# antoyang/FrozenBiLM

Measured on AMD Instinct MI355X. Metric: video-text samples/sec (MLM fwd+bwd) DeBERTa-XL+adapters, higher is better.
Workload: dtype bf16; 1 GPU; DeBERTa-v2-XLarge(24L)+adapters ds8/8, B=32/GPU, T=10x1024, L=256 (S=266), MLM fwd+bwd+allreduce+clip+Adam, dropout 0.1 live, seeded random weights; global_batch=32, seq_len=266, parallelism=dp1, dead_layer23_encoder_pass=skipped (output unused, SURVEY fact 6); FLOPs still counted

## Files before the change

frozenbilm_amd/csrc/attn_bwd.hip:

```cpp
#include "attn_common.h"
#include "../../include/fbl.h"

namespace {
using namespace attn;

__global__ void rowdot_kernel(const bf16* dO, const bf16* O, long ld, float* out, int B, int S, int nh) {
  const long gid = (long)blockIdx.x * blockDim.x + threadIdx.x;
  const long idx = gid >> 3;
  const int c = (int)(gid & 7);
  const long total = (long)B * S * nh;
  const bool live = idx < total;
  const long row = live ? idx / nh : 0;
  const int h = live ? (int)(idx % nh) : 0;
  float s = 0.f;
  if (live) {
    const bf16x8 x = *(const bf16x8*)(dO + row * ld + h * 64 + c * 8);
    const bf16x8 y = *(const bf16x8*)(O + row * ld + h * 64 + c * 8);
#pragma unroll
    for (int e = 0; e < 8; ++e) s += bf2f(x[e]) * bf2f(y[e]);
  }
  s += __shfl_xor(s, 1, 64);
  s += __shfl_xor(s, 2, 64);
  s += __shfl_xor(s, 4, 64);
  if (live && c == 0) {
// ... 643 lines not shown
      *(bf16x4*)(ok + dt * 16) = (bf16x4){f2bf(dk[dt][0]), f2bf(dk[dt][1]), f2bf(dk[dt][2]), f2bf(dk[dt][3])};
    }
  }
}

struct BwdQArgs {
  const bf16* dS;
  const bf16* k; long ldk;
  const bf16* pkx;
  const int32_t* klen; const int32_t* border;
  bf16* dQ; long lddq;
  int B, S, Sp, nh;
  const int32_t* row0;
};
constexpr int LDG1 = 104;
constexpr int Q_DS = 0;
constexpr int Q_KS = Q_DS + 8192;
constexpr int Q_G1 = Q_KS + 8192;
constexpr int Q_TAB = Q_G1 + 64 * LDG1 * 2;
constexpr int Q_TOTAL = Q_TAB + 16384;
static_assert(3 * Q_TOTAL <= 160 * 1024, "three workgroups per CU");

template <bool PACKED = false>
__global__ __launch_bounds__(256, 3) void attn_bwd_dq_kernel(BwdQArgs a) {
  extern __shared__ __attribute__((aligned(16))) char smem[];
  const int tid = threadIdx.x, lane = tid & 63;
  const int w = __builtin_amdgcn_readfirstlane(tid >> 6);
  const int c = lane & 15, g = lane >> 4;
  const int S = a.S, Sp = a.Sp;
  const WgCoord wc = wg_coord(Sp / 64, a.nh, a.B, a.border);
  const int i0 = wc.x * 64, h = wc.h, b = wc.b;
  const int i = i0 + w * 16 + c;
  const long rb = PACKED ? (long)a.row0[b] : (long)b * S;
  const int lim = PACKED ? min(a.row0[b + 1] - a.row0[b], S) : S;
  const int kl = a.klen ? min(a.klen[b], S) : S;
  const int nkt = (i0 < kl) ? (kl + 63) / 64 : 0;
  const int srow = tid >> 3, sch = tid & 7;
  const int sb = srow * 128 + ((sch ^ tswz(srow)) << 4);
  const int ks0 = (w < 2) ? 0 : 1;
  bf16* g1 = (bf16*)(smem + Q_G1) + (w * 16 + c) * LDG1;
  const int wr = w * 16 + c;
  f32x4 dq[4];
#pragma unroll
  for (int dt = 0; dt < 4; ++dt) dq[dt] = (f32x4){0.f, 0.f, 0.f, 0.f};
  if (nkt > 0) {
    for (int t = tid; t < (64 * LDG1 * 2) / 16; t += 256) *(bf16x8*)(smem + Q_G1 + t * 16) = (bf16x8){0, 0, 0, 0, 0, 0, 0, 0};
    __syncthreads();
  }

  const long sbase = ((long)b * a.nh + h) * Sp * Sp;
  const __amdgpu_buffer_rsrc_t sr = buf_rsrc(a.dS + sbase + (long)i0 * Sp);
  const __amdgpu_buffer_rsrc_t kr = buf_rsrc(a.k + rb * a.ldk + h * 64);
  const __amdgpu_buffer_rsrc_t xr = buf_rsrc(a.pkx + (long)h * 2 * Sp * 64);
  const uint32_t so = (uint32_t)((wr * Sp + g * 16) * 2);
  const uint32_t ldk2 = (uint32_t)(a.ldk * 2);
  const int beta0 = (i0 - 64 + Sp) >> 6;

  struct Regs { bf16x8 s[2], k[2], x[2]; } R;
  auto load_pair = [&](int jt) {
#pragma unroll
    for (int t = 0; t < 2; ++t) {
      R.s[t] = buf_ld16(sr, so + (uint32_t)(t * 16), (uint32_t)(jt * 128));
      const uint32_t jr = (uint32_t)min(jt * 64 + srow + t * 32, lim - 1);
      R.k[t] = buf_ld16(kr, jr * ldk2 + (uint32_t)(sch * 16), 0);
      R.x[t] = buf_ld16(xr, (uint32_t)((srow + t * 32) * 128 + sch * 16), (uint32_t)((beta0 - jt) * 8192));
    }
  };
  if (nkt > 0) {
    load_pair(0);
#pragma unroll
    for (int t = 0; t < 2; ++t)
      *(bf16x8*)(smem + Q_TAB + ((beta0 + 1) & 1) * 8192 + sb + t * 4096) =
          buf_ld16(xr, (uint32_t)((srow + t * 32) * 128 + sch * 16), (uint32_t)((beta0 + 1) * 8192));
  }
  for (int jt = 0; jt < nkt; ++jt) {
#pragma unroll
    for (int t = 0; t < 2; ++t) {
      *(bf16x8*)(smem + Q_KS + sb + t * 4096) = R.k[t];
      *(bf16x8*)(smem + Q_TAB + ((beta0 - jt) & 1) * 8192 + sb + t * 4096) = R.x[t];
      *(bf16x8*)(smem + Q_DS + wr * 128 + (((2 * g + t) ^ (wr & 7)) << 4)) = R.s[t];
    }
    {
      bf16* gs = g1 + wr + 64 - g * 16 - ks0 * 32;
#pragma unroll
      for (int t = 0; t < 2; ++t)
#pragma unroll
        for (int e = 0; e < 8; ++e) gs[-(t * 8 + e)] = R.s[t][e];
    }
    __syncthreads();
    load_pair(min(jt + 1, nkt - 1));
#pragma unroll
    for (int kk = 0; kk < 2; ++kk) {
      const int rk = kk * 32 + g * 8 + (c >> 2);
      const bf16x8 sf = *(const bf16x8*)(smem + Q_DS + wr * 128 + (((kk * 4 + g) ^ (wr & 7)) << 4));
#pragma unroll
      for (int dt = 0; dt < 4; ++dt) {
        const int ch = dt * 2 + ((c >> 1) & 1), sub = (c & 1) * 8;
        union { tr16x4 h[2]; bf16x8 v; } u;
        u.h[0] = lds_tr16((const bf16*)(smem + Q_KS + rk * 128 + ((ch ^ tswz(rk)) << 4) + sub));
        u.h[1] = lds_tr16((const bf16*)(smem + Q_KS + (rk + 4) * 128 + ((ch ^ tswz(rk + 4)) << 4) + sub));
        dq[dt] = __builtin_amdgcn_mfma_f32_16x16x32_bf16(u.v, sf, dq[dt], 0, 0, 0);
      }
    }
#pragma unroll
    for (int u3 = 0; u3 < 3; ++u3) {
      const int x0 = (ks0 + u3) * 32 + g * 8;
      const int slot = ((beta0 - jt + (x0 >> 6)) & 1) * 8192;
      const int r = (x0 & 63) + (c >> 2);
      const bf16x8 gf = *(const bf16x8*)(g1 + u3 * 32 + g * 8);
#pragma unroll
      for (int dt = 0; dt < 4; ++dt) {
        const int ch = dt * 2 + ((c >> 1) & 1), sub = (c & 1) * 8;
        union { tr16x4 h[2]; bf16x8 v; } ut;
        ut.h[0] = lds_tr16((const bf16*)(smem + Q_TAB + slot + r * 128 + ((ch ^ tswz(r)) << 4) + sub));
        ut.h[1] = lds_tr16((const bf16*)(smem + Q_TAB + slot + (r + 4) * 128 + ((ch ^ tswz(r + 4)) << 4) + sub));
        dq[dt] = __builtin_amdgcn_mfma_f32_16x16x32_bf16(ut.v, gf, dq[dt], 0, 0, 0);
      }
    }
    __syncthreads();
  }
  if (i < lim) {
    bf16* op = a.dQ + (rb + i) * a.lddq + h * 64 + g * 4;
#pragma unroll
    for (int dt = 0; dt < 4; ++dt)
      *(bf16x4*)(op + dt * 16) = (bf16x4){f2bf(dq[dt][0]), f2bf(dq[dt][1]), f2bf(dq[dt][2]), f2bf(dq[dt][3])};
  }
}

struct ShearArgs {
  const bf16* X;
  const bf16* YT; long y_sh, y_sb, y_sd;
  const bf16* PT;
  const int16_t* relidx;
  const int32_t* klen;
  const int32_t* border;
  bf16* out; long ldout;
  int B, S, Sp, nh, span2, Wg;
  int lin;
  const int32_t* row0;
};
__device__ __forceinline__ void gt_window(const int16_t* relidx, int S, int kl, int r0, int Wg, int* rbase, int* nks) {
  const int hi = 2 * S - 2;
  const int dlo = -(r0 + 31), dhi = kl - 1 - r0;
  const int rb = (int)relidx[min(max(dlo + S - 1, 0), hi)] & ~7;
  const int rt = (int)relidx[min(max(dhi + S - 1, 0), hi)];
  *rbase = rb;
  *nks = min((rt - rb + 32) / 32, Wg / 32);
}
constexpr int C_IDX = 0;
constexpr int C_G = C_IDX + 2048;

template <bool PACKED = false>
__global__ __launch_bounds__(128) void attn_bwd_shear_kernel(ShearArgs a) {
  extern __shared__ __attribute__((aligned(16))) char smem[];
  const int tid = threadIdx.x, lane = tid & 63;
  const int w = __builtin_amdgcn_readfirstlane(tid >> 6);
  const int c = lane & 15, g = lane >> 4;
  const int S = a.S, Sp = a.Sp;
  const WgCoord wc = wg_coord(Sp / 32, a.nh, a.B, a.border);
  const int r0 = wc.x * 32, h = wc.h, b = wc.b;
  const int LDG = a.Wg + 8;
  const int rl = w * 16 + c;
  const int row = r0 + rl;
  bf16* G = (bf16*)(smem + C_G);
  int16_t* idx = (int16_t*)(smem + C_IDX);
  const bf16x8 z8 = {0, 0, 0, 0, 0, 0, 0, 0};
  const int kl = a.klen ? min(a.klen[b], S) : S;
  const long rb = PACKED ? (long)a.row0[b] : (long)b * S;
  const int lim = PACKED ? min(a.row0[b + 1] - a.row0[b], S) : S;
  if (r0 >= kl) {
    if (row < lim) {
      bf16* op = a.out + (rb + row) * a.ldout + h * 64 + g * 4;
#pragma unroll
      for (int dt = 0; dt < 4; ++dt) *(bf16x4*)(op + dt * 16) = (bf16x4){0, 0, 0, 0};
    }
    return;
  }
  int rbase, nks;
  gt_window(a.relidx, S, kl, r0, a.Wg, &rbase, &nks);
  const int izero = (int)a.relidx[S - 1];
  {
    const int vpr = nks * 4;
    for (int t = tid; t < 32 * vpr; t += 128) *(bf16x8*)(G + (t / vpr) * LDG + (t % vpr) * 8) = z8;
  }
  attn::load_idx_padded(idx, a.relidx, S, Sp, tid, 128);
  const long xbase = (((long)b * a.nh + h) * Sp + row) * Sp;
  f32x4 acc[4];
#pragma unroll
  for (int dt = 0; dt < 4; ++dt) acc[dt] = (f32x4){0.f, 0.f, 0.f, 0.f};
  __syncthreads();

  const int nct = (kl + 63) / 64;
  const bf16* ytb = a.YT + h * a.y_sh + b * a.y_sb + (long)c * a.y_sd + g * 8;
  const int16_t* ib = idx + (Sp - 1 - row + g * 8);
  bf16* grow = G + rl * LDG - rbase;
  const int wmax = rbase + nks * 32 - 1;
  const int dummy = rbase + a.Wg;
  const int lin0 = izero + g * 8 - row;
  const int rw = r0 + w * 16;
  struct Frags { bf16x8 y[8], x[2]; };
  auto load_ct = [&](int ct, Frags& F) {
    const int c0 = ct * 64;
#pragma unroll
    for (int kk = 0; kk < 2; ++kk)
#pragma unroll
      for (int dt = 0; dt < 4; ++dt)
        F.y[kk * 4 + dt] = (FBL_ATTN_DBGBITS & 2048) ? z8 : *(const bf16x8*)(ytb + (long)(dt * 16) * a.y_sd + c0 + kk * 32);
    F.x[0] = *(const bf16x8*)(a.X + xbase + c0 + g * 8);
    F.x[1] = *(const bf16x8*)(a.X + xbase + c0 + 32 + g * 8);
  };
  auto step = [&](int ct, const Frags& F) {
    const int c0 = ct * 64;
    const int d_a = rw - (c0 + 63), d_b = rw + 15 - c0;
    const bool band = max(abs(d_a), abs(d_b)) < a.lin;
#pragma unroll
    for (int kk = 0; kk < 2; ++kk) {
      const bf16x8 xv = F.x[kk];
#pragma unroll
      for (int dt = 0; dt < 4; ++dt) acc[dt] = __builtin_amdgcn_mfma_f32_16x16x32_bf16(F.y[kk * 4 + dt], xv, acc[dt], 0, 0, 0);
      const int cb = c0 + kk * 32;
      if (FBL_ATTN_DBGBITS & 512) continue;
      if (band) {
        const int s0 = lin0 + cb;
#pragma unroll
        for (int e = 0; e < 8; ++e) {
          const int slot = s0 + e;
          grow[bf2f(xv[e]) != 0.f ? slot : dummy] = xv[e];
        }
      } else {
#pragma unroll
        for (int e = 0; e < 8; ++e) {
          const float x = bf2f(xv[e]);
          if (x != 0.f) {
            const int dlt = cb + g * 8 + e - row;
            const int gi = clampi((int)ib[cb + e], rbase, wmax);
            if (abs(dlt) < a.lin) {
              grow[gi] = xv[e];
            } else {
              bf16x2 pv = {(bf16)0.f, (bf16)0.f};
              pv[gi & 1] = xv[e];
              __builtin_amdgcn_ds_atomic_fadd_v2bf16((__attribute__((address_space(3))) bf16x2*)(grow + (gi & ~1)), pv);
            }
          }
        }
      }
    }
  };
  {
    Frags F0, F1;
    load_ct(0, F0);
    for (int ct = 0; ct < nct; ct += 2) {
      if (ct + 1 < nct) load_ct(ct + 1, F1);
      step(ct, F0);
      if (ct + 2 < nct) load_ct(ct + 2, F0);
      if (ct + 1 < nct) step(ct + 1, F1);
    }
  }
  const bf16* pt = a.PT + (long)h * 64 * a.span2 + rbase + g * 8;
  auto load_pt = [&](int kk, bf16x8* dstf) {
#pragma unroll
    for (int dt = 0; dt < 4; ++dt) {
      const bool ok = rbase + kk * 32 + g * 8 + 8 <= a.span2;
      dstf[dt] = ok ? *(const bf16x8*)(pt + (long)(dt * 16 + c) * a.span2 + kk * 32) : z8;
    }
  };
  auto table_step = [&](int kk, const bf16x8* af) {
    const bf16x8 bfv = *(const bf16x8*)(G + rl * LDG + kk * 32 + g * 8);
#pragma unroll
    for (int dt = 0; dt < 4; ++dt) acc[dt] = __builtin_amdgcn_mfma_f32_16x16x32_bf16(af[dt], bfv, acc[dt], 0, 0, 0);
  };
  bf16x8 pa[4], pb[4];
  const int nks_run = (FBL_ATTN_DBGBITS & 1024) ? 0 : nks;
  load_pt(0, pa);
  for (int kk = 0; kk < nks_run; kk += 2) {
    if (kk + 1 < nks) load_pt(kk + 1, pb);
    table_step(kk, pa);
    if (kk + 2 < nks) load_pt(kk + 2, pa);
    if (kk + 1 < nks) table_step(kk + 1, pb);
  }
  if (row < lim) {
    bf16* op = a.out + (rb + row) * a.ldout + h * 64 + g * 4;
#pragma unroll
    for (int dt = 0; dt < 4; ++dt)
      *(bf16x4*)(op + dt * 16) = (bf16x4){f2bf(acc[dt][0]), f2bf(acc[dt][1]), f2bf(acc[dt][2]), f2bf(acc[dt][3])};
  }
}

constexpr int PG_MAX_E = 64;
struct PosGradArgs {
  const bf16* X[PG_MAX_E];
  const bf16* Y[PG_MAX_E];
  long ldy;
  const int16_t* dlo;
  const int16_t* dcnt;
  const int32_t* klen;
  const int32_t* row0;
  float* out;
  int E, B, S, Sp, nh, rcnt;
  int cmax;
};
constexpr int PG_PAD = 48;
constexpr int PG_LDY = 80;
constexpr int PG_TPW = 4;
constexpr int PG_WAVES = 4, PG_THR = PG_WAVES * 64;
constexpr int PG_ROWS = PG_WAVES * PG_TPW * 16;
__host__ __device__ constexpr int pg_pitch(int Sp) { return Sp + 2 * PG_PAD; }
__host__ __device__ constexpr int pg_buf(int Sp) { return 32 * pg_pitch(Sp) * 2 + 32 * PG_LDY * 2; }
__host__ __device__ constexpr int pg_smem(int Sp) { return 2 * pg_buf(Sp); }

template <bool NEG, int CM, int NXR, int OCC>
__global__ __launch_bounds__(PG_THR, OCC) void pos_grad_kernel(PosGradArgs a) {
  extern __shared__ __attribute__((aligned(16))) char smem[];
  const int tid = threadIdx.x, lane = tid & 63;
  const int w = __builtin_amdgcn_readfirstlane(tid >> 6);
  const int c = lane & 15, g = lane >> 4;
  const int S = a.S, Sp = a.Sp, P = pg_pitch(Sp);
  const int nsplit = (a.rcnt + PG_ROWS - 1) / PG_ROWS;
  const int L8 = blockIdx.x >> 3, xcd = blockIdx.x & 7;
  const int prob = (L8 / nsplit) * 8 + xcd, part = L8 % nsplit;
  if (prob >= a.E * a.nh) return;
  const int e = prob / a.nh, h = prob % a.nh;
  const int bufsz = pg_buf(Sp);
  const bf16* X = a.X[e];
  const bf16* Y = a.Y[e];
  const int ntiles = (a.rcnt + 15) / 16;

  int d0[PG_TPW], dn[PG_TPW], tlo[PG_TPW], thi[PG_TPW];
  bool simple[PG_TPW];
#pragma unroll
  for (int u = 0; u < PG_TPW; ++u) {
    const int t = (w + PG_WAVES * u) * nsplit + part;
    const int r = min(t * 16 + c, a.rcnt - 1);
    const bool live = t < ntiles && t * 16 + c < a.rcnt;
    d0[u] = live ? (int)a.dlo[r] : 0;
    dn[u] = live ? (int)a.dcnt[r] : 0;
    const int rf = min(t * 16, a.rcnt - 1), rl = min(t * 16 + 15, a.rcnt - 1);
    tlo[u] = t < ntiles ? (int)a.dlo[rf] : 1 << 20;
    thi[u] = t < ntiles ? (int)a.dlo[rl] + (int)a.dcnt[rl] - 1 : -(1 << 20);
    simple[u] = t < ntiles && t * 16 + 15 < a.rcnt && (thi[u] - tlo[u]) == 15 && __builtin_amdgcn_ballot_w64(dn[u] != 1) == 0;
  }
  f32x4 acc[PG_TPW][4];
#pragma unroll
  for (int u = 0; u < PG_TPW; ++u)
#pragma unroll
    for (int dt = 0; dt < 4; ++dt) acc[u][dt] = (f32x4){0.f, 0.f, 0.f, 0.f};

  for (int id = tid; id < (OCC >= 3 ? 1 : 2) * 32 * 2 * (PG_PAD / 8); id += PG_THR) {
    const int bsel = id / (32 * 2 * (PG_PAD / 8)), r2 = id % (32 * 2 * (PG_PAD / 8));
    const int row = r2 / (2 * (PG_PAD / 8)), q = r2 % (2 * (PG_PAD / 8));
    const int col = q < PG_PAD / 8 ? q * 8 : PG_PAD + Sp + (q - PG_PAD / 8) * 8;
    *(bf16x8*)((bf16*)(smem + bsel * bufsz) + row * P + col) = (bf16x8){0, 0, 0, 0, 0, 0, 0, 0};
  }
  const bf16x8 z8 = (bf16x8){0, 0, 0, 0, 0, 0, 0, 0};
  const int srow = tid >> 3, sch = tid & 7, nq = Sp >> 6;

  int b_n = 0, k_n = 0, kl_n = 0;
  auto seek = [&]() {
    while (b_n < a.B) {
      kl_n = a.klen ? min(a.klen[b_n], S) : S;
      if (k_n < kl_n) return true;
      ++b_n; k_n = 0;
    }
    return false;
  };
  bf16x8 rx[NXR], ry;
  int it_b = 0, it_k = 0, it_kl = 0;
  auto load_item = [&]() {
    it_b = b_n; it_k = k_n; it_kl = kl_n;
    const int kl64 = (kl_n + 63) & ~63;
    const long rb = a.row0 ? (long)a.row0[b_n] : (long)b_n * S;
    const int lim = a.row0 ? min(a.row0[b_n + 1] - a.row0[b_n], S) : S;
    const bf16* Xb = X + (((long)b_n * a.nh + h) * Sp) * Sp + (long)k_n * Sp;
    const bf16* xr = Xb + (long)srow * Sp + sch * 8;
#pragma unroll
    for (int q = 0; q < NXR; ++q) rx[q] = (q < nq && sch * 8 + q * 64 < kl64) ? *(const bf16x8*)(xr + q * 64) : z8;
    {
      const int pos = k_n + srow;
      ry = (pos < lim) ? *(const bf16x8*)(Y + (rb + pos) * a.ldy + h * 64 + sch * 8) : z8;
    }
    k_n += 32;
  };
  int pb = 0;
  bool have = seek();
  if (have) load_item();
  while (have) {
    bf16* xs = (bf16*)(smem + pb * bufsz);
    bf16* ys = xs + 32 * P;
    if (OCC >= 3) __syncthreads();
    {
      bf16* xw = xs + srow * P + PG_PAD + sch * 8;
#pragma unroll
      for (int q = 0; q < NXR; ++q)
        if (q < nq) *(bf16x8*)(xw + q * 64) = rx[q];
    }
    *(bf16x8*)(ys + srow * PG_LDY + sch * 8) = ry;
    const int k0 = it_k, kl = it_kl;
    __syncthreads();
    have = seek();
    if (have) load_item();
    bf16x8 yf[4];
#pragma unroll
    for (int dt = 0; dt < 4; ++dt) {
      const bf16* yb = ys + (g * 8 + (c >> 2)) * PG_LDY + dt * 16 + (c & 3) * 4;
      union { tr16x4 hh[2]; bf16x8 v; } u2;
      u2.hh[0] = lds_tr16(yb);
      u2.hh[1] = lds_tr16(yb + 4 * PG_LDY);
      yf[dt] = u2.v;
    }
#pragma unroll
    for (int u = 0; u < PG_TPW; ++u) {
      const int cmin = NEG ? k0 + tlo[u] : k0 - thi[u];
      const int cmax = NEG ? k0 + 31 + thi[u] : k0 + 31 - tlo[u];
      if (cmax < 0 || cmin >= kl) continue;
      bf16x8 gf;
      const bf16* xrow = xs + (g * 8) * P + PG_PAD;
      const int cb = NEG ? (k0 + g * 8 + d0[u]) : (k0 + g * 8 - d0[u]);
      if (simple[u]) {
#pragma unroll
        for (int q = 0; q < 8; ++q) gf[q] = xrow[q * P + cb + q];
      } else {
        const int lo = -PG_PAD, hi = Sp + PG_PAD - 1;
        bf16 vv[8][CM];
#pragma unroll
        for (int q = 0; q < 8; ++q)
#pragma unroll
          for (int t2 = 0; t2 < CM; ++t2) vv[q][t2] = xrow[q * P + clampi(NEG ? cb + q + t2 : cb + q - t2, lo, hi)];
#pragma unroll
        for (int q = 0; q < 8; ++q) {
          float sum = 0.f;
#pragma unroll
          for (int t2 = 0; t2 < CM; ++t2) sum += t2 < dn[u] ? bf2f(vv[q][t2]) : 0.f;
          gf[q] = f2bf(sum);
        }
      }
#pragma unroll
      for (int dt = 0; dt < 4; ++dt) acc[u][dt] = __builtin_amdgcn_mfma_f32_16x16x32_bf16(yf[dt], gf, acc[u][dt], 0, 0, 0);
    }
    if (OCC < 3) pb ^= 1;
  }
  float* ob = a.out + ((long)e * a.nh + h) * a.rcnt * 64;
#pragma unroll
  for (int u = 0; u < PG_TPW; ++u) {
    const int r = ((w + PG_WAVES * u) * nsplit + part) * 16 + c;
    if (r < a.rcnt) {
#pragma unroll
      for (int dt = 0; dt < 4; ++dt) *(f32x4*)(ob + (long)r * 64 + dt * 16 + g * 4) = acc[u][dt];
    }
  }
}

constexpr int PGW_PAD = 6;
__host__ __device__ constexpr int pgw_pitch(int Sp) { return Sp + PGW_PAD; }
__host__ __device__ constexpr int pgw_smem(int Sp) { return 32 * pgw_pitch(Sp) * 4 + 32 * PG_LDY * 2; }

template <bool NEG>
__global__ __launch_bounds__(PG_THR, 2) void pos_grad_wide_kernel(PosGradArgs a) {
  extern __shared__ __attribute__((aligned(16))) char smem[];
  const int tid = threadIdx.x, lane = tid & 63;
  const int w = __builtin_amdgcn_readfirstlane(tid >> 6);
  const int c = lane & 15, g = lane >> 4;
  const int S = a.S, Sp = a.Sp, PP = pgw_pitch(Sp);
  const int nsplit = (a.rcnt + PG_ROWS - 1) / PG_ROWS;
  const int L8 = blockIdx.x >> 3, xcd = blockIdx.x & 7;
  const int prob = (L8 / nsplit) * 8 + xcd, part = L8 % nsplit;
  if (prob >= a.E * a.nh) return;
  const int e = prob / a.nh, h = prob % a.nh;
  float* cs = (float*)smem;
  bf16* ys = (bf16*)(smem + 32 * PP * 4);
  const bf16* X = a.X[e];
  const bf16* Y = a.Y[e];
  const int ntiles = (a.rcnt + 15) / 16;

  int d0[PG_TPW], dn[PG_TPW], tlo[PG_TPW], thi[PG_TPW];
#pragma unroll
  for (int u = 0; u < PG_TPW; ++u) {
    const int t = (w + PG_WAVES * u) * nsplit + part;
    const int r = min(t * 16 + c, a.rcnt - 1);
    const bool live = t < ntiles && t * 16 + c < a.rcnt;
    d0[u] = live ? (int)a.dlo[r] : 0;
    dn[u] = live ? (int)a.dcnt[r] : 0;
    const int rf = min(t * 16, a.rcnt - 1), rl = min(t * 16 + 15, a.rcnt - 1);
    tlo[u] = t < ntiles ? (int)a.dlo[rf] : 1 << 20;
    thi[u] = t < ntiles ? (int)a.dlo[rl] + (int)a.dcnt[rl] - 1 : -(1 << 20);
  }
  f32x4 acc[PG_TPW][4];
#pragma unroll
  for (int u = 0; u < PG_TPW; ++u)
#pragma unroll
    for (int dt = 0; dt < 4; ++dt) acc[u][dt] = (f32x4){0.f, 0.f, 0.f, 0.f};

  if (tid < 32) cs[tid * PP + 1] = 0.f;
  const bf16x8 z8 = (bf16x8){0, 0, 0, 0, 0, 0, 0, 0};
  const int srow = tid >> 3, sch = tid & 7, nq = Sp >> 6;

  int b_n = 0, k_n = 0, kl_n = 0;
  auto seek = [&]() {
    while (b_n < a.B) {
      kl_n = a.klen ? min(a.klen[b_n], S) : S;
      if (k_n < kl_n) return true;
      ++b_n; k_n = 0;
    }
    return false;
  };
  bf16x8 rx[8], ry;
  int it_k = 0, it_kl = 0;
  auto load_item = [&]() {
    it_k = k_n; it_kl = kl_n;
    const int kl64 = (kl_n + 63) & ~63;
    const long rb = a.row0 ? (long)a.row0[b_n] : (long)b_n * S;
    const int lim = a.row0 ? min(a.row0[b_n + 1] - a.row0[b_n], S) : S;
    const bf16* xr = X + (((long)b_n * a.nh + h) * Sp) * Sp + (long)(k_n + srow) * Sp + sch * 8;
#pragma unroll
    for (int q = 0; q < 8; ++q) rx[q] = (q < nq && sch * 8 + q * 64 < kl64) ? *(const bf16x8*)(xr + q * 64) : z8;
    const int pos = k_n + srow;
    ry = (pos < lim) ? *(const bf16x8*)(Y + (rb + pos) * a.ldy + h * 64 + sch * 8) : z8;
    k_n += 32;
  };
  bool have = seek();
  if (have) load_item();
  while (have) {
    __syncthreads();
    {
      float* cw = cs + srow * PP + 2 + sch * 8;
      float carry = 0.f;
#pragma unroll
      for (int q = 0; q < 8; ++q) {
        if (q < nq) {
          float run[8];
          run[0] = bf2f(rx[q][0]);
#pragma unroll
          for (int i = 1; i < 8; ++i) run[i] = run[i - 1] + bf2f(rx[q][i]);
          float incl = run[7];
#pragma unroll
          for (int s = 1; s < 8; s <<= 1) {
            const float o = __shfl_up(incl, s, 8);
            if (sch >= s) incl += o;
          }
          const float excl = __shfl_up(incl, 1, 8);
          const float base = carry + (sch ? excl : 0.f);
#pragma unroll
          for (int i = 0; i < 8; i += 2) *(float2*)(cw + q * 64 + i) = make_float2(base + run[i], base + run[i + 1]);
          carry += __shfl(incl, 7, 8);
        }
      }
    }
    *(bf16x8*)(ys + srow * PG_LDY + sch * 8) = ry;
    const int k0 = it_k, kl = it_kl;
    __syncthreads();
    have = seek();
    if (have) load_item();
    bf16x8 yf[4];
#pragma unroll
    for (int dt = 0; dt < 4; ++dt) {
      const bf16* yb = ys + (g * 8 + (c >> 2)) * PG_LDY + dt * 16 + (c & 3) * 4;
      union { tr16x4 hh[2]; bf16x8 v; } u2;
      u2.hh[0] = lds_tr16(yb);
      u2.hh[1] = lds_tr16(yb + 4 * PG_LDY);
      yf[dt] = u2.v;
    }
    const float* crow = cs + (g * 8) * PP + 1;
#pragma unroll
    for (int u = 0; u < PG_TPW; ++u) {
      const int cmin = NEG ? k0 + tlo[u] : k0 - thi[u];
      const int cmax = NEG ? k0 + 31 + thi[u] : k0 + 31 - tlo[u];
      if (cmax < 0 || cmin >= kl) continue;
      const int kb = k0 + g * 8;
      float hi[8], lo[8];
#pragma unroll
      for (int q = 0; q < 8; ++q) {
        const int jl = NEG ? kb + q + d0[u] : kb + q - d0[u] - dn[u] + 1;
        hi[q] = crow[q * PP + clampi(jl + dn[u], 0, Sp)];
        lo[q] = crow[q * PP + clampi(jl, 0, Sp)];
      }
      bf16x8 gf;
#pragma unroll
      for (int q = 0; q < 8; ++q) gf[q] = f2bf(hi[q] - lo[q]);
#pragma unroll
      for (int dt = 0; dt < 4; ++dt) acc[u][dt] = __builtin_amdgcn_mfma_f32_16x16x32_bf16(yf[dt], gf, acc[u][dt], 0, 0, 0);
    }
  }
  float* ob = a.out + ((long)e * a.nh + h) * a.rcnt * 64;
#pragma unroll
  for (int u = 0; u < PG_TPW; ++u) {
    const int r = ((w + PG_WAVES * u) * nsplit + part) * 16 + c;
    if (r < a.rcnt) {
#pragma unroll
      for (int dt = 0; dt < 4; ++dt) *(f32x4*)(ob + (long)r * 64 + dt * 16 + g * 4) = acc[u][dt];
    }
  }
}

}

extern "C" int fbl_attn_rowdot(const void* dO, const void* O, int64_t ld, float* out, int B, int S, int nh,
                               void* stream) {
  if (ld % 8) return FBL_ERR_ALIGN;
  const long total = (long)B * S * nh;
  if (total <= 0) return 0;
  hipLaunchKernelGGL(rowdot_kernel, dim3((unsigned)((total * 8 + 255) / 256)), dim3(256), 0, (hipStream_t)stream,
                     (const bf16*)dO, (const bf16*)O, (long)ld, out, B, S, nh);
  FBL_CHECK_LAUNCH();
  return 0;
}

extern "C" int fbl_disent_attn_bwd_ds(const void* q, const void* k, const void* v, int64_t ldq, const void* dO,
                                      int64_t ldo,
                                      const void* pk, const void* pq, int64_t ldp, const int16_t* relidx,
                                      const int32_t* mask, const int32_t* klen, const int32_t* border, const float* lse, const float* Dv, float scale, float p_drop,
                                      uint64_t seed, const uint64_t* seed_dev, void* dV, int64_t lddv, void* dS, void* dST, int B, int S, int Sp,
                                      int nh, int span2, int lin_span, const int32_t* row0, void* stream) {
  if (S < 1 || S > 512 || Sp < S || Sp % 64) return FBL_ERR_SHAPE;
  if ((ldq % 8) || (ldo % 8) || (ldp % 8) || (lddv % 4)) return FBL_ERR_ALIGN;
  if (lin_span < 0 || 2 * lin_span > span2) return FBL_ERR_ARG;
  if (row0 && !klen) return FBL_ERR_ARG;
  if (B <= 0 || nh <= 0) return 0;
  BwdAArgs a{(const bf16*)q, (const bf16*)k, (const bf16*)v, ldq, (const bf16*)dO, ldo, (const bf16*)pk, (const bf16*)pq, ldp, relidx, mask, klen, border, lse, Dv, scale, p_drop, seed, (bf16*)dV, lddv,
             (bf16*)dS, (bf16*)dST, B, S, Sp, nh, span2, lin_span, seed_dev, row0};
  attn_debug_init();
  const int smem_bytes = a_total(Sp);
  static int attr_bytes = 0;
  if (smem_bytes > attr_bytes) {
    hipError_t e = hipFuncSetAttribute((const void*)attn_bwd_ds_kernel<false>, hipFuncAttributeMaxDynamicSharedMemorySize, smem_bytes);
    if (e == hipSuccess) e = hipFuncSetAttribute((const void*)attn_bwd_ds_kernel<true>, hipFuncAttributeMaxDynamicSharedMemorySize, smem_bytes);
    if (e == hipSuccess) e = hipFuncSetAttribute((const void*)attn_bwd_ds_kernel<false, true>, hipFuncAttributeMaxDynamicSharedMemorySize, smem_bytes);
    if (e == hipSuccess) e = hipFuncSetAttribute((const void*)attn_bwd_ds_kernel<true, true>, hipFuncAttributeMaxDynamicSharedMemorySize, smem_bytes);
    if (e != hipSuccess) return (int)e;
    attr_bytes = smem_bytes;
  }
  const dim3 grid((unsigned)(Sp / 64) * nh * B);
  const bool devseed = seed_dev && p_drop > 0.f;
  if (row0 && devseed)
    hipLaunchKernelGGL((attn_bwd_ds_kernel<true, true>), grid, dim3(256), smem_bytes, (hipStream_t)stream, a);
  else if (row0)
    hipLaunchKernelGGL((attn_bwd_ds_kernel<false, true>), grid, dim3(256), smem_bytes, (hipStream_t)stream, a);
  else if (devseed)
    hipLaunchKernelGGL(attn_bwd_ds_kernel<true>, grid, dim3(256), smem_bytes, (hipStream_t)stream, a);
  else
    hipLaunchKernelGGL(attn_bwd_ds_kernel<false>, grid, dim3(256), smem_bytes, (hipStream_t)stream, a);
  FBL_CHECK_LAUNCH();
  return 0;
}

extern "C" int fbl_disent_attn_bwd_dspk(const void* psave, const float* msave, const void* q, int64_t ldq, const void* v, int64_t ldv,
                                        const void* dO, int64_t ldo, const void* pqx, const int32_t* klen, const int32_t* border,
                                        const float* lse, const float* Dv, float scale, float p_drop, uint64_t seed,
                                        const uint64_t* seed_dev, void* dK, int64_t lddk, void* dV, int64_t lddv, void* dS, void* dST,
                                        int B, int S, int Sp, int nh, const int32_t* row0, void* stream) {
  if (S < 1 || S > 512 || Sp < S || Sp % 64) return FBL_ERR_SHAPE;
  if ((ldv % 8) || (ldo % 8) || (ldq % 8) || (lddv % 4) || (lddk % 4)) return FBL_ERR_ALIGN;
  if (!psave || !msave || !q || !v || !dO || !pqx || !lse || !Dv || !dK || !dV || !dS || !dST) return FBL_ERR_ARG;
  if (row0 && !klen) return FBL_ERR_ARG;
  if (B <= 0 || nh <= 0) return 0;
  BwdPKArgs a{{(const bf16*)psave, msave, (const bf16*)v, ldv, (const bf16*)dO, ldo, klen, border, lse, Dv, scale, p_drop, seed,
               seed_dev, (bf16*)dV, lddv, (bf16*)dS, (bf16*)dST, B, S, Sp, nh, row0},
              (const bf16*)q, ldq, (const bf16*)pqx, (bf16*)dK, lddk};
  attn_debug_init();
  static bool attr_set = false;
  if (!attr_set) {
    hipError_t e = hipFuncSetAttribute((const void*)attn_bwd_dspk_kernel<false>, hipFuncAttributeMaxDynamicSharedMemorySize, K_TOTAL);
    if (e == hipSuccess) e = hipFuncSetAttribute((const void*)attn_bwd_dspk_kernel<true>, hipFuncAttributeMaxDynamicSharedMemorySize, K_TOTAL);
    if (e != hipSuccess) return (int)e;
    attr_set = true;
  }
  const dim3 grid((unsigned)(Sp / 64) * nh * B);
  if (row0)
    hipLaunchKernelGGL(attn_bwd_dspk_kernel<true>, grid, dim3(256), K_TOTAL, (hipStream_t)stream, a);
  else
    hipLaunchKernelGGL(attn_bwd_dspk_kernel<false>, grid, dim3(256), K_TOTAL, (hipStream_t)stream, a);
  FBL_CHECK_LAUNCH();
  return 0;
}

extern "C" int fbl_disent_attn_bwd_dq(const void* dS, const void* k, int64_t ldk, const void* pkx, const int32_t* klen,
                                      const int32_t* border, void* dQ, int64_t lddq, int B, int S, int Sp, int nh,
                                      const int32_t* row0, void* stream) {
  if (S < 1 || S > 512 || Sp < S || Sp % 64) return FBL_ERR_SHAPE;
  if ((ldk % 8) || (lddq % 4)) return FBL_ERR_ALIGN;
  if (!dS || !k || !pkx || !dQ) return FBL_ERR_ARG;
  if (row0 && !klen) return FBL_ERR_ARG;
  if (B <= 0 || nh <= 0) return 0;
  BwdQArgs a{(const bf16*)dS, (const bf16*)k, ldk, (const bf16*)pkx, klen, border, (bf16*)dQ, lddq, B, S, Sp, nh, row0};
  static bool attr_set = false;
  if (!attr_set) {
    hipError_t e = hipFuncSetAttribute((const void*)attn_bwd_dq_kernel<false>, hipFuncAttributeMaxDynamicSharedMemorySize, Q_TOTAL);
    if (e == hipSuccess) e = hipFuncSetAttribute((const void*)attn_bwd_dq_kernel<true>, hipFuncAttributeMaxDynamicSharedMemorySize, Q_TOTAL);
    if (e != hipSuccess) return (int)e;
    attr_set = true;
  }
  const dim3 grid((unsigned)(Sp / 64) * nh * B);
  if (row0)
    hipLaunchKernelGGL(attn_bwd_dq_kernel<true>, grid, dim3(256), Q_TOTAL, (hipStream_t)stream, a);
  else
    hipLaunchKernelGGL(attn_bwd_dq_kernel<false>, grid, dim3(256), Q_TOTAL, (hipStream_t)stream, a);
  FBL_CHECK_LAUNCH();
  return 0;
}

extern "C" int fbl_disent_attn_bwd_shear(const void* dST, const void* QT, int64_t y_sh, int64_t y_sb, int64_t y_sd,
                                         const void* PQT, const int16_t* relidx, const int32_t* klen, const int32_t* border,
                                         void* dK, int64_t lddk, int lin_span, int B, int S, int Sp, int nh, int span2,
                                         const int32_t* row0, void* stream) {
  if (S < 1 || S > 512 || Sp < S || Sp % 64 || span2 > 512 || span2 % 32) return FBL_ERR_SHAPE;
  if ((lddk % 4) || (y_sd % 8) || (y_sb % 8) || (y_sh % 8)) return FBL_ERR_ALIGN;
  if (B <= 0 || nh <= 0) return 0;
  int Wg = S + 31 + 7;
  if (Wg > span2) Wg = span2;
  Wg = (Wg + 31) / 32 * 32;
  if (row0 && !klen) return FBL_ERR_ARG;
  ShearArgs a{(const bf16*)dST, (const bf16*)QT, y_sh, y_sb, y_sd, (const bf16*)PQT, relidx, klen, border, (bf16*)dK, lddk,
              B, S, Sp, nh, span2, Wg, lin_span, row0};
  attn_debug_init();
  const int smem_bytes = C_G + 32 * (Wg + 8) * 2;
  static int attr_bytes = 0;
  if (smem_bytes > attr_bytes) {
    hipError_t e = hipFuncSetAttribute((const void*)attn_bwd_shear_kernel<false>, hipFuncAttributeMaxDynamicSharedMemorySize, smem_bytes);
    if (e == hipSuccess) e = hipFuncSetAttribute((const void*)attn_bwd_shear_kernel<true>, hipFuncAttributeMaxDynamicSharedMemorySize, smem_bytes);
    if (e != hipSuccess) return (int)e;
    attr_bytes = smem_bytes;
  }
  dim3 grid((unsigned)(Sp / 32) * nh * B);
  if (row0)
    hipLaunchKernelGGL(attn_bwd_shear_kernel<true>, grid, dim3(128), smem_bytes, (hipStream_t)stream, a);
  else
    hipLaunchKernelGGL(attn_bwd_shear_kernel<false>, grid, dim3(128), smem_bytes, (hipStream_t)stream, a);
  FBL_CHECK_LAUNCH();
  return 0;
}

extern "C" int fbl_attn_pos_grad(int neg, const void* const* X, const void* const* Y, int64_t ldy, const int16_t* dlo,
                                 const int16_t* dcnt, int dcnt_max, const int32_t* klen, const int32_t* row0, float* out, int E,
                                 int B, int S, int Sp, int nh, int rcnt, void* stream) {
  if (S < 1 || S > 512 || Sp < S || Sp % 64 || rcnt < 1 || rcnt > 1024) return FBL_ERR_SHAPE;
  if (ldy % 8) return FBL_ERR_ALIGN;
  if (!X || !Y || !dlo || !dcnt || !out || dcnt_max < 1) return FBL_ERR_ARG;
  if (row0 && !klen) return FBL_ERR_ARG;
  if (E <= 0 || B <= 0 || nh <= 0) return 0;
  for (int e = 0; e < E; ++e)
    if (!X[e] || !Y[e]) return FBL_ERR_ARG;
  static const int occ_sw = FBL_ENV_INT("FBL_POSGRAD_OCC", 3);
  const bool occ3 = Sp <= 320 && dcnt_max <= 3 && occ_sw >= 3;
  const int smem_bytes = occ3 ? pg_buf(Sp) : pg_smem(Sp);
  static int attr_bytes = 0;
  if (pg_smem(Sp) > attr_bytes) {
    const void* fns[6] = {(const void*)pos_grad_kernel<false, 3, 5, 3>, (const void*)pos_grad_kernel<true, 3, 5, 3>,
                          (const void*)pos_grad_kernel<false, 3, 8, 2>, (const void*)pos_grad_kernel<true, 3, 8, 2>,
                          (const void*)pos_grad_kernel<false, 8, 8, 2>, (const void*)pos_grad_kernel<true, 8, 8, 2>};
    for (int i = 0; i < 6; ++i) {
      hipError_t e1 = hipFuncSetAttribute(fns[i], hipFuncAttributeMaxDynamicSharedMemorySize, pg_smem(Sp));
      if (e1 != hipSuccess) return (int)e1;
    }
    attr_bytes = pg_smem(Sp);
  }
  const bool wide = dcnt_max > 8;
  static int attr_wide = 0;
  if (wide && pgw_smem(Sp) > attr_wide) {
    for (const void* fn : {(const void*)pos_grad_wide_kernel<false>, (const void*)pos_grad_wide_kernel<true>}) {
      hipError_t e1 = hipFuncSetAttribute(fn, hipFuncAttributeMaxDynamicSharedMemorySize, pgw_smem(Sp));
      if (e1 != hipSuccess) return (int)e1;
    }
    attr_wide = pgw_smem(Sp);
  }
  const int nsplit = (rcnt + PG_ROWS - 1) / PG_ROWS;
  for (int e0 = 0; e0 < E; e0 += PG_MAX_E) {
    PosGradArgs a{};
    const int ne = E - e0 < PG_MAX_E ? E - e0 : PG_MAX_E;
    for (int e = 0; e < ne; ++e) {
      a.X[e] = (const bf16*)X[e0 + e];
      a.Y[e] = (const bf16*)Y[e0 + e];
    }
    a.ldy = ldy; a.dlo = dlo; a.dcnt = dcnt; a.klen = klen; a.row0 = row0;
    a.out = out + (long)e0 * nh * rcnt * 64;
    a.E = ne; a.B = B; a.S = S; a.Sp = Sp; a.nh = nh; a.rcnt = rcnt; a.cmax = dcnt_max;
    const dim3 grid((unsigned)(((ne * nh + 7) / 8) * 8 * nsplit));
#define FBL_PG_LAUNCH(NEG_, CM_, NXR_, OCC_) \
  hipLaunchKernelGGL((pos_grad_kernel<NEG_, CM_, NXR_, OCC_>), grid, dim3(PG_THR), smem_bytes, (hipStream_t)stream, a)
    if (wide) {
      if (neg) hipLaunchKernelGGL(pos_grad_wide_kernel<true>, grid, dim3(PG_THR), pgw_smem(Sp), (hipStream_t)stream, a);
      else hipLaunchKernelGGL(pos_grad_wide_kernel<false>, grid, dim3(PG_THR), pgw_smem(Sp), (hipStream_t)stream, a);
    } else if (occ3) {
      if (neg) FBL_PG_LAUNCH(true, 3, 5, 3);
      else FBL_PG_LAUNCH(false, 3, 5, 3);
    } else if (dcnt_max <= 3) {
      if (neg) FBL_PG_LAUNCH(true, 3, 8, 2);
      else FBL_PG_LAUNCH(false, 3, 8, 2);
    } else {
      if (neg) FBL_PG_LAUNCH(true, 8, 8, 2);
      else FBL_PG_LAUNCH(false, 8, 8, 2);
    }
#undef FBL_PG_LAUNCH
    FBL_CHECK_LAUNCH();
  }
  return 0;
}

extern "C" int fbl_attn_bwd_prep(const void* q, int64_t ldq, const void* pq, const void* pk, int64_t ldp, const void* dO,
                                 const void* O, int64_t ldo, void* QT, void* PQT, float* Dv, const int16_t* relidx, void* PQX,
                                 void* PKX, int B, int S, int Sp, int nh, int span2, const int32_t* row0, void* stream) {
  if (S < 1 || Sp < S || Sp % 64 || span2 <= 0 || span2 % 64) return FBL_ERR_SHAPE;
  if ((ldq % 8) || (ldp % 8) || (ldo % 8)) return FBL_ERR_ALIGN;
  if ((PQX || PKX) && !relidx) return FBL_ERR_ARG;
  if (!Dv) return FBL_ERR_ARG;
  if (B <= 0 || nh <= 0) return 0;
  const int n_tr = (Sp / 64) * nh * B, n_tab = (span2 / 64) * nh, n_x = (2 * Sp / 64) * nh;
  PrepArgs a{(const bf16*)q, ldq, (const bf16*)pq, (const bf16*)pk, ldp, (const bf16*)dO, (const bf16*)O, ldo, (bf16*)QT,
             (bf16*)PQT, Dv, B, S, Sp, nh, span2, QT ? n_tr : 0, PQT ? n_tab : 0, row0, relidx, (bf16*)PQX, (bf16*)PKX,
             PQX ? n_x : 0, PKX ? n_x : 0};
  const long n_dot = ((long)B * S * nh * 8 + 255) / 256;
  const long grid = (long)a.n_qt + a.n_pqt + a.n_pqx + a.n_pkx + n_dot;
  hipLaunchKernelGGL(attn_bwd_prep_kernel, dim3((unsigned)grid), dim3(256), 0, (hipStream_t)stream, a);
  FBL_CHECK_LAUNCH();
  return 0;
}
```

Measured before the change: 773.0 samples/s.

## Add 6-tile-per-wave pos_grad variant with LDS metadata and key-block skipping

Adds a TPW=6 template variant of the relative-position gradient kernel, used when rcnt fits in one split. Each block then covers all rows with contiguous tile assignment, stores per-row delta metadata in LDS to relieve register pressure, and skips key blocks whose diagonal range cannot touch the block's rows. It also makes global loads unconditional via clamped addresses, masking at the LDS store, and uses a fixed pitch under occupancy 3. These changes trade more work per block and extra LDS for fewer blocks, less redundant X/Y loading and fewer branches, at the risk of lower parallelism for the grid.

```diff
diff --git a/frozenbilm_amd/csrc/attn_bwd.hip b/frozenbilm_amd/csrc/attn_bwd.hip
--- a/frozenbilm_amd/csrc/attn_bwd.hip
+++ b/frozenbilm_amd/csrc/attn_bwd.hip
@@ -969,46 +969,62 @@
 constexpr int PG_PAD = 48;
 constexpr int PG_LDY = 80;
 constexpr int PG_TPW = 4;
+constexpr int PG_TPW1 = 6;
 constexpr int PG_WAVES = 4, PG_THR = PG_WAVES * 64;
 constexpr int PG_ROWS = PG_WAVES * PG_TPW * 16;
+constexpr int PG_ROWS1 = PG_WAVES * PG_TPW1 * 16;
+constexpr int PG_RCNT1 = PG_ROWS1 + PG_WAVES * 16;
 __host__ __device__ constexpr int pg_pitch(int Sp) { return Sp + 2 * PG_PAD; }
 __host__ __device__ constexpr int pg_buf(int Sp) { return 32 * pg_pitch(Sp) * 2 + 32 * PG_LDY * 2; }
 __host__ __device__ constexpr int pg_smem(int Sp) { return 2 * pg_buf(Sp); }
-
-template <bool NEG, int CM, int NXR, int OCC>
+__host__ __device__ constexpr int pg_meta(int tpw) { return tpw > PG_TPW ? PG_WAVES * tpw * 16 * 4 : 0; }
+__host__ __device__ constexpr int pg_pitch_fixed(int nxr, int occ, int tpw) {
+  return (tpw > PG_TPW && occ >= 3) ? pg_pitch(nxr * 64) : 0;
+}
+
+template <bool NEG, int CM, int NXR, int OCC, int TPW>
 __global__ __launch_bounds__(PG_THR, OCC) void pos_grad_kernel(PosGradArgs a) {
   extern __shared__ __attribute__((aligned(16))) char smem[];
   const int tid = threadIdx.x, lane = tid & 63;
   const int w = __builtin_amdgcn_readfirstlane(tid >> 6);
   const int c = lane & 15, g = lane >> 4;
-  const int S = a.S, Sp = a.Sp, P = pg_pitch(Sp);
-  const int nsplit = (a.rcnt + PG_ROWS - 1) / PG_ROWS;
+  constexpr int ROWS = PG_WAVES * TPW * 16;
+  constexpr bool LMETA = pg_meta(TPW) > 0;
+  constexpr int PFIX = pg_pitch_fixed(NXR, OCC, TPW);
+  const int S = a.S, Sp = a.Sp, P = PFIX ? PFIX : pg_pitch(Sp);
+  const int nsplit = (a.rcnt + ROWS - 1) / ROWS;
   const int L8 = blockIdx.x >> 3, xcd = blockIdx.x & 7;
   const int prob = (L8 / nsplit) * 8 + xcd, part = L8 % nsplit;
   if (prob >= a.E * a.nh) return;
   const int e = prob / a.nh, h = prob % a.nh;
-  const int bufsz = pg_buf(Sp);
+  const int bufsz = 32 * P * 2 + 32 * PG_LDY * 2;
   const bf16* X = a.X[e];
   const bf16* Y = a.Y[e];
   const int ntiles = (a.rcnt + 15) / 16;
 
-  int d0[PG_TPW], dn[PG_TPW], tlo[PG_TPW], thi[PG_TPW];
-  bool simple[PG_TPW];
-#pragma unroll
-  for (int u = 0; u < PG_TPW; ++u) {
-    const int t = (w + PG_WAVES * u) * nsplit + part;
+  auto uni = [](int v) { return LMETA ? __builtin_amdgcn_readfirstlane(v) : v; };
+  int d0[TPW], dn[TPW], tlo[TPW], thi[TPW];
+  bool simple[TPW];
+  int* meta = (int*)(smem + (OCC >= 3 ? 1 : 2) * bufsz) + w * 16 + c;
+#pragma unroll
+  for (int u = 0; u < TPW; ++u) {
+    const int t = LMETA ? part * (PG_WAVES * TPW) + w + PG_WAVES * u : (w + PG_WAVES * u) * nsplit + part;
     const int r = min(t * 16 + c, a.rcnt - 1);
     const bool live = t < ntiles && t * 16 + c < a.rcnt;
     d0[u] = live ? (int)a.dlo[r] : 0;
     dn[u] = live ? (int)a.dcnt[r] : 0;
     const int rf = min(t * 16, a.rcnt - 1), rl = min(t * 16 + 15, a.rcnt - 1);
-    tlo[u] = t < ntiles ? (int)a.dlo[rf] : 1 << 20;
-    thi[u] = t < ntiles ? (int)a.dlo[rl] + (int)a.dcnt[rl] - 1 : -(1 << 20);
+    tlo[u] = uni(t < ntiles ? (int)a.dlo[rf] : 1 << 20);
+    thi[u] = uni(t < ntiles ? (int)a.dlo[rl] + (int)a.dcnt[rl] - 1 : -(1 << 20));
     simple[u] = t < ntiles && t * 16 + 15 < a.rcnt && (thi[u] - tlo[u]) == 15 && __builtin_amdgcn_ballot_w64(dn[u] != 1) == 0;
-  }
-  f32x4 acc[PG_TPW][4];
-#pragma unroll
-  for (int u = 0; u < PG_TPW; ++u)
+    if (LMETA) {
+      simple[u] = uni(simple[u] && __builtin_amdgcn_ballot_w64(d0[u] != tlo[u] + c) == 0) != 0;
+      meta[u * 64] = (d0[u] & 0xffff) | (dn[u] << 16);
+    }
+  }
+  f32x4 acc[TPW][4];
+#pragma unroll
+  for (int u = 0; u < TPW; ++u)
 #pragma unroll
     for (int dt = 0; dt < 4; ++dt) acc[u][dt] = (f32x4){0.f, 0.f, 0.f, 0.f};
 
@@ -1020,31 +1036,42 @@
   }
   const bf16x8 z8 = (bf16x8){0, 0, 0, 0, 0, 0, 0, 0};
   const int srow = tid >> 3, sch = tid & 7, nq = Sp >> 6;
-
+  unsigned xoff = __umul24(srow, Sp) + sch * 8;
+  asm volatile("" : "+v"(xoff));
+
+  int plo = 0, phi = 0;
+  if (LMETA) {
+    const int rf = min(part * ROWS, a.rcnt - 1), rl = min(part * ROWS + ROWS - 1, a.rcnt - 1);
+    plo = uni((int)a.dlo[rf]);
+    phi = uni((int)a.dlo[rl] + (int)a.dcnt[rl] - 1);
+  }
   int b_n = 0, k_n = 0, kl_n = 0;
   auto seek = [&]() {
     while (b_n < a.B) {
-      kl_n = a.klen ? min(a.klen[b_n], S) : S;
+      kl_n = uni(a.klen ? min(a.klen[b_n], S) : S);
+      if (LMETA) {
+        while (k_n < kl_n && ((NEG ? k_n + 31 + phi : k_n + 31 - plo) < 0 || (NEG ? k_n + plo : k_n - phi) >= kl_n)) k_n += 32;
+      }
       if (k_n < kl_n) return true;
       ++b_n; k_n = 0;
     }
     return false;
   };
   bf16x8 rx[NXR], ry;
-  int it_b = 0, it_k = 0, it_kl = 0;
+  int it_k = 0, it_kl = 0, it_lim = 0;
   auto load_item = [&]() {
-    it_b = b_n; it_k = k_n; it_kl = kl_n;
+    it_k = k_n; it_kl = kl_n;
     const int kl64 = (kl_n + 63) & ~63;
-    const long rb = a.row0 ? (long)a.row0[b_n] : (long)b_n * S;
-    const int lim = a.row0 ? min(a.row0[b_n + 1] - a.row0[b_n], S) : S;
+    const long rb = a.row0 ? (long)uni(a.row0[b_n]) : (long)b_n * S;
+    it_lim = uni(a.row0 ? min(a.row0[b_n + 1] - a.row0[b_n], S) : S);
+    unsigned xo = xoff;
+    asm volatile("" : "+v"(xo));
+    const int rlast = max(it_lim - 1, 0), kb = min(k_n, rlast);
+    const unsigned yo = __umul24(min(srow, rlast - kb), (unsigned)a.ldy) + sch * 8;
     const bf16* Xb = X + (((long)b_n * a.nh + h) * Sp) * Sp + (long)k_n * Sp;
-    const bf16* xr = Xb + (long)srow * Sp + sch * 8;
-#pragma unroll
-    for (int q = 0; q < NXR; ++q) rx[q] = (q < nq && sch * 8 + q * 64 < kl64) ? *(const bf16x8*)(xr + q * 64) : z8;
-    {
-      const int pos = k_n + srow;
-      ry = (pos < lim) ? *(const bf16x8*)(Y + (rb + pos) * a.ldy + h * 64 + sch * 8) : z8;
-    }
+#pragma unroll
+    for (int q = 0; q < NXR; ++q) rx[q] = *(const bf16x8*)(Xb + xo + min(q * 64, kl64 - 64));
+    ry = *(const bf16x8*)(Y + ((it_lim > 0 ? rb : 0) + kb) * a.ldy + h * 64 + yo);
     k_n += 32;
   };
   int pb = 0;
@@ -1056,11 +1083,12 @@
     if (OCC >= 3) __syncthreads();
     {
       bf16* xw = xs + srow * P + PG_PAD + sch * 8;
+      const int kl64 = (it_kl + 63) & ~63;
 #pragma unroll
       for (int q = 0; q < NXR; ++q)
-        if (q < nq) *(bf16x8*)(xw + q * 64) = rx[q];
-    }
-    *(bf16x8*)(ys + srow * PG_LDY + sch * 8) = ry;
+        if (q < nq) *(bf16x8*)(xw + q * 64) = q * 64 < kl64 ? rx[q] : z8;
+    }
+    *(bf16x8*)(ys + srow * PG_LDY + sch * 8) = it_k + srow < it_lim ? ry : z8;
     const int k0 = it_k, kl = it_kl;
     __syncthreads();
     have = seek();
@@ -1074,30 +1102,46 @@
       u2.hh[1] = lds_tr16(yb + 4 * PG_LDY);
       yf[dt] = u2.v;
     }
-#pragma unroll
-    for (int u = 0; u < PG_TPW; ++u) {
+    int gc = NEG ? g * 8 + c : g * 8 - c;
+    if (LMETA) asm volatile("" : "+v"(gc));
+    const int kc = k0 + gc;
+#pragma unroll
+    for (int u = 0; u < TPW; ++u) {
       const int cmin = NEG ? k0 + tlo[u] : k0 - thi[u];
       const int cmax = NEG ? k0 + 31 + thi[u] : k0 + 31 - tlo[u];
       if (cmax < 0 || cmin >= kl) continue;
       bf16x8 gf;
       const bf16* xrow = xs + (g * 8) * P + PG_PAD;
-      const int cb = NEG ? (k0 + g * 8 + d0[u]) : (k0 + g * 8 - d0[u]);
       if (simple[u]) {
+        const int cb = LMETA ? (NEG ? kc + tlo[u] : kc - tlo[u]) : (NEG ? (k0 + g * 8 + d0[u]) : (k0 + g * 8 - d0[u]));
 #pragma unroll
         for (int q = 0; q < 8; ++q) gf[q] = xrow[q * P + cb + q];
       } else {
+        int d0u = d0[u], dnu = dn[u];
+        if (LMETA) {
+          const int m = meta[u * 64];
+          d0u = (int)(short)m; dnu = m >> 16;
+        }
+        const int cb = NEG ? (k0 + g * 8 + d0u) : (k0 + g * 8 - d0u);
         const int lo = -PG_PAD, hi = Sp + PG_PAD - 1;
-        bf16 vv[8][CM];
-#pragma unroll
-        for (int q = 0; q < 8; ++q)
-#pragma unroll
-          for (int t2 = 0; t2 < CM; ++t2) vv[q][t2] = xrow[q * P + clampi(NEG ? cb + q + t2 : cb + q - t2, lo, hi)];
-#pragma unroll
-        for (int q = 0; q < 8; ++q) {
-          float sum = 0.f;
-#pragma unroll
-          for (int t2 = 0; t2 < CM; ++t2) sum += t2 < dn[u] ? bf2f(vv[q][t2]) : 0.f;
-          gf[q] = f2bf(sum);
+        constexpr int QC = LMETA ? 4 : 8;
+#pragma unroll
+        for (int q0 = 0; q0 < 8; q0 += QC) {
+          bf16 vv[QC][CM];
+#pragma unroll
+          for (int q = 0; q < QC; ++q)
+#pragma unroll
+            for (int t2 = 0; t2 < CM; ++t2) {
+              const int col = clampi(NEG ? cb + q0 + q + t2 : cb + q0 + q - t2, lo, hi);
+              vv[q][t2] = xrow[(q0 + q) * P + ((LMETA && t2 >= dnu) ? lo : col)];
+            }
+#pragma unroll
+          for (int q = 0; q < QC; ++q) {
+            float sum = 0.f;
+#pragma unroll
+            for (int t2 = 0; t2 < CM; ++t2) sum += (LMETA || t2 < dnu) ? bf2f(vv[q][t2]) : 0.f;
+            gf[q0 + q] = f2bf(sum);
+          }
         }
       }
 #pragma unroll
@@ -1106,12 +1150,15 @@
     if (OCC < 3) pb ^= 1;
   }
   float* ob = a.out + ((long)e * a.nh + h) * a.rcnt * 64;
-#pragma unroll
-  for (int u = 0; u < PG_TPW; ++u) {
-    const int r = ((w + PG_WAVES * u) * nsplit + part) * 16 + c;
+  int ln = 0;
+  asm volatile("" : "+v"(ln));
+  ln = __builtin_amdgcn_mbcnt_hi(~0u, __builtin_amdgcn_mbcnt_lo(~0u, ln));
+#pragma unroll
+  for (int u = 0; u < TPW; ++u) {
+    const int r = (LMETA ? part * (PG_WAVES * TPW) + w + PG_WAVES * u : (w + PG_WAVES * u) * nsplit + part) * 16 + (ln & 15);
     if (r < a.rcnt) {
 #pragma unroll
-      for (int dt = 0; dt < 4; ++dt) *(f32x4*)(ob + (long)r * 64 + dt * 16 + g * 4) = acc[u][dt];
+      for (int dt = 0; dt < 4; ++dt) *(f32x4*)(ob + (long)r * 64 + dt * 16 + (ln >> 4) * 4) = acc[u][dt];
     }
   }
 }
@@ -1399,6 +1446,7 @@
                                  int B, int S, int Sp, int nh, int rcnt, void* stream) {
   if (S < 1 || S > 512 || Sp < S || Sp % 64 || rcnt < 1 || rcnt > 1024) return FBL_ERR_SHAPE;
   if (ldy % 8) return FBL_ERR_ALIGN;
+  if (ldy < 64 || ldy >= (1 << 24)) return FBL_ERR_SHAPE;
   if (!X || !Y || !dlo || !dcnt || !out || dcnt_max < 1) return FBL_ERR_ARG;
   if (row0 && !klen) return FBL_ERR_ARG;
   if (E <= 0 || B <= 0 || nh <= 0) return 0;
@@ -1406,17 +1454,22 @@
     if (!X[e] || !Y[e]) return FBL_ERR_ARG;
   static const int occ_sw = FBL_ENV_INT("FBL_POSGRAD_OCC", 3);
   const bool occ3 = Sp <= 320 && dcnt_max <= 3 && occ_sw >= 3;
-  const int smem_bytes = occ3 ? pg_buf(Sp) : pg_smem(Sp);
+  const bool one = rcnt <= PG_RCNT1;
+  const int smem_bytes = (occ3 ? pg_buf(one ? 5 * 64 : Sp) : pg_smem(Sp)) + (one ? pg_meta(PG_TPW1) : 0);
   static int attr_bytes = 0;
-  if (pg_smem(Sp) > attr_bytes) {
-    const void* fns[6] = {(const void*)pos_grad_kernel<false, 3, 5, 3>, (const void*)pos_grad_kernel<true, 3, 5, 3>,
-                          (const void*)pos_grad_kernel<false, 3, 8, 2>, (const void*)pos_grad_kernel<true, 3, 8, 2>,
-                          (const void*)pos_grad_kernel<false, 8, 8, 2>, (const void*)pos_grad_kernel<true, 8, 8, 2>};
-    for (int i = 0; i < 6; ++i) {
-      hipError_t e1 = hipFuncSetAttribute(fns[i], hipFuncAttributeMaxDynamicSharedMemorySize, pg_smem(Sp));
+  const int smem_max = (pg_smem(Sp) > pg_buf(5 * 64) ? pg_smem(Sp) : pg_buf(5 * 64)) + pg_meta(PG_TPW1);
+  if (smem_max > attr_bytes) {
+#define FBL_PG_FNS(TPW_) \
+  (const void*)pos_grad_kernel<false, 3, 5, 3, TPW_>, (const void*)pos_grad_kernel<true, 3, 5, 3, TPW_>, \
+  (const void*)pos_grad_kernel<false, 3, 8, 2, TPW_>, (const void*)pos_grad_kernel<true, 3, 8, 2, TPW_>, \
+  (const void*)pos_grad_kernel<false, 8, 8, 2, TPW_>, (const void*)pos_grad_kernel<true, 8, 8, 2, TPW_>
+    const void* fns[12] = {FBL_PG_FNS(PG_TPW), FBL_PG_FNS(PG_TPW1)};
+#undef FBL_PG_FNS
+    for (int i = 0; i < 12; ++i) {
+      hipError_t e1 = hipFuncSetAttribute(fns[i], hipFuncAttributeMaxDynamicSharedMemorySize, smem_max);
       if (e1 != hipSuccess) return (int)e1;
     }
-    attr_bytes = pg_smem(Sp);
+    attr_bytes = smem_max;
   }
   const bool wide = dcnt_max > 8;
   static int attr_wide = 0;
@@ -1427,7 +1480,8 @@
     }
     attr_wide = pgw_smem(Sp);
   }
-  const int nsplit = (rcnt + PG_ROWS - 1) / PG_ROWS;
+  const int nsplit_w = (rcnt + PG_ROWS - 1) / PG_ROWS;
+  const int nsplit = one ? (rcnt + PG_ROWS1 - 1) / PG_ROWS1 : nsplit_w;
   for (int e0 = 0; e0 < E; e0 += PG_MAX_E) {
     PosGradArgs a{};
     const int ne = E - e0 < PG_MAX_E ? E - e0 : PG_MAX_E;
@@ -1438,9 +1492,14 @@
     a.ldy = ldy; a.dlo = dlo; a.dcnt = dcnt; a.klen = klen; a.row0 = row0;
     a.out = out + (long)e0 * nh * rcnt * 64;
     a.E = ne; a.B = B; a.S = S; a.Sp = Sp; a.nh = nh; a.rcnt = rcnt; a.cmax = dcnt_max;
-    const dim3 grid((unsigned)(((ne * nh + 7) / 8) * 8 * nsplit));
-#define FBL_PG_LAUNCH(NEG_, CM_, NXR_, OCC_) \
-  hipLaunchKernelGGL((pos_grad_kernel<NEG_, CM_, NXR_, OCC_>), grid, dim3(PG_THR), smem_bytes, (hipStream_t)stream, a)
+    const dim3 grid((unsigned)(((ne * nh + 7) / 8) * 8 * (wide ? nsplit_w : nsplit)));
+#define FBL_PG_LAUNCH(NEG_, CM_, NXR_, OCC_)                                                                                  \
+  do {                                                                                                                        \
+    if (one)                                                                                                                  \
+      hipLaunchKernelGGL((pos_grad_kernel<NEG_, CM_, NXR_, OCC_, PG_TPW1>), grid, dim3(PG_THR), smem_bytes, (hipStream_t)stream, a); \
+    else                                                                                                                      \
+      hipLaunchKernelGGL((pos_grad_kernel<NEG_, CM_, NXR_, OCC_, PG_TPW>), grid, dim3(PG_THR), smem_bytes, (hipStream_t)stream, a);  \
+  } while (0)
     if (wide) {
       if (neg) hipLaunchKernelGGL(pos_grad_wide_kernel<true>, grid, dim3(PG_THR), pgw_smem(Sp), (hipStream_t)stream, a);
       else hipLaunchKernelGGL(pos_grad_wide_kernel<false>, grid, dim3(PG_THR), pgw_smem(Sp), (hipStream_t)stream, a);
```

Result: no change. 776.4 samples/s, median of 4 (+0.4%).
